# jin-s13/GKGNet

Measured on AMD Instinct MI355X. Metric: Grapher fwd+bwd images/sec, higher is better.
Workload: dtype f32; 1 GPU; BASELINE cfg2-literal: Grapher(C320,G4,k9,d1,18x18,relpos)+GrapherLabel(L80) fwd+bwd; batch_per_gpu=32, global_batch=32, C=320, G=4, HW=18x18, k=9, dilation=1, bn=local, parallelism=dp1, input_layout=nchw, launch=hipGraph replay of fwd+bwd+grad-pack, world_size=1, backend=none (single process), grad_allreduce=none (1 GPU)

## Files before the change

### gkgnet_amd/csrc/gkg_gemm_x6.hip

```cpp
#include "gkg_common.h"
#include <stdlib.h>
#include <vector>

namespace gkg {

typedef float x6_f32x16 __attribute__((ext_vector_type(16)));
typedef __attribute__((__vector_size__(8 * sizeof(__bf16)))) __bf16 x6_bf16x8;
typedef __bf16 x6_bf16x2 __attribute__((ext_vector_type(2)));
typedef float x6_f32x2 __attribute__((ext_vector_type(2)));

constexpr int X6_NPAD = 128;

__device__ __forceinline__ unsigned x6_cvt2(float a, float b) {
  x6_f32x2 v = {a, b};
  return __builtin_bit_cast(unsigned, __builtin_convertvector(v, x6_bf16x2));
}

__device__ __forceinline__ void x6_split2(float x0, float x1, unsigned& h, unsigned& m, unsigned& l) {
  h = x6_cvt2(x0, x1);
  const float r0 = x0 - __uint_as_float(h << 16), r1 = x1 - __uint_as_float(h & 0xffff0000u);
  m = x6_cvt2(r0, r1);
  const float s0 = r0 - __uint_as_float(m << 16), s1 = r1 - __uint_as_float(m & 0xffff0000u);
  l = x6_cvt2(s0, s1);
}
// ... 407 lines not shown
         ((flags & GKG_X6_FORCE_KS) || (nb == 1 && N <= 640));
}

static int x6_tile_ksplit(long long base2, int nk_total, bool has_ws) {
  if (!has_ws || base2 >= 320 || nk_total < 8) return 1;
  int ks = (int)(X6_SK_MAX_WG / base2);
  if (ks > nk_total / 4) ks = nk_total / 4;
  return ks > 8 ? 8 : ks;
}

template <int EPI>
static hipError_t x6_launch(X6Args a, int nb, hipStream_t st, void* sk_ws = nullptr, size_t sk_bytes = 0, unsigned flags = 0) {
  GkgProfScope prof(GKG_PROF_GEMM_X6, st, 2.0 * a.M * a.N * a.K * nb);
  const int mt = (a.M + 127) / 128;
  const long long base2 = (long long)mt * ((a.N + 63) / 64) * nb;
  const int nk_total = (a.K + 31) / 32;
  if constexpr (EPI != X6_STORE_NCHW) {
    if (x6_ks_form(a.M, a.N, nb, sk_ws != nullptr, flags)) {
      return x6_launch_ks<EPI, 1>(a, nb, st);
    }
  }
  if (const int ks = x6_tile_ksplit(base2, nk_total, sk_ws && sk_bytes >= X6_SK_BYTES); ks >= 2) {
    a.kper = (nk_total + ks - 1) / ks;
    a.ksplit = (nk_total + a.kper - 1) / a.kper;
    a.cnt = reinterpret_cast<unsigned*>(sk_ws);
    a.part = reinterpret_cast<float*>(reinterpret_cast<char*>(sk_ws) + X6_SK_CNT_BYTES);
    return x6_launch_ni<2, EPI>(a, nb, st);
  }
  if constexpr (EPI == X6_BNBWD) {
    if (a.add) return hipErrorInvalidValue;
  }
  int ni = base2 < 160 && !(flags & GKG_X6_FORCE_WALK) ? 1 : 2;
  if constexpr (EPI != X6_BNBWD && EPI != X6_STORE_NCHW) {
    if (a.N == 80 && ni == 2) return x6_launch_ni<3, EPI, 80>(a, nb, st);
  }
  if (ni == 1) return x6_launch_ni<1, EPI>(a, nb, st);
  if constexpr (EPI == X6_BNBWD) return x6_launch_ni<2, EPI>(a, nb, st);
  else return x6_launch_ni<2, EPI, 64, true>(a, nb, st, flags);
}

struct X6WgradArgs {
  const float* A;  size_t a_bstride;  int lda;
  const float* B;  size_t b_bstride;  int ldb;
  float* C;  size_t c_bstride;  int ldc;
  int M, N, K;
  int mtiles, ntiles, splits, rows_per_split;
  int swap;
  int share, rot;
  int ubase, urem;
  int kperm;
};

typedef unsigned x6_u32x4 __attribute__((ext_vector_type(4)));
typedef x6_u32x4 X6WFrag[4][3];

__device__ __forceinline__ x6_bf16x8 x6w_operand(const x6_u32x4& f) { return __builtin_bit_cast(x6_bf16x8, f); }
template <int I>
__device__ __forceinline__ void x6w_op(float (&raw)[4][8], X6WFrag& fn, unsigned (&t0)[4], unsigned (&t1)[4]) {
  constexpr int blk = I / 44, u = I % 44, p = u & 3, o = u >> 2;
  float& x0 = raw[blk][2 * p]; float& x1 = raw[blk][2 * p + 1];
  unsigned w;
  if constexpr (o == 0) { asm volatile("v_cvt_pk_bf16_f32 %0, %1, %2" : "=v"(w) : "v"(x0), "v"(x1)); fn[blk][0][p] = w; }
  if constexpr (o == 1) asm volatile("v_lshlrev_b32 %0, 16, %1" : "=v"(t0[p]) : "v"(fn[blk][0][p]));
  if constexpr (o == 2) asm volatile("v_and_b32 %0, 0xffff0000, %1" : "=v"(t1[p]) : "v"(fn[blk][0][p]));
  if constexpr (o == 3) asm volatile("v_sub_f32 %0, %0, %1" : "+v"(x0) : "v"(t0[p]));
  if constexpr (o == 4) asm volatile("v_sub_f32 %0, %0, %1" : "+v"(x1) : "v"(t1[p]));
  if constexpr (o == 5) { asm volatile("v_cvt_pk_bf16_f32 %0, %1, %2" : "=v"(w) : "v"(x0), "v"(x1)); fn[blk][1][p] = w; }
  if constexpr (o == 6) asm volatile("v_lshlrev_b32 %0, 16, %1" : "=v"(t0[p]) : "v"(fn[blk][1][p]));
  if constexpr (o == 7) asm volatile("v_and_b32 %0, 0xffff0000, %1" : "=v"(t1[p]) : "v"(fn[blk][1][p]));
  if constexpr (o == 8) asm volatile("v_sub_f32 %0, %0, %1" : "+v"(x0) : "v"(t0[p]));
  if constexpr (o == 9) asm volatile("v_sub_f32 %0, %0, %1" : "+v"(x1) : "v"(t1[p]));
  if constexpr (o == 10) { asm volatile("v_cvt_pk_bf16_f32 %0, %1, %2" : "=v"(w) : "v"(x0), "v"(x1)); fn[blk][2][p] = w; }
}
template <int I, int END>
__device__ __forceinline__ void x6w_ops(float (&raw)[4][8], X6WFrag& fn, unsigned (&t0)[4], unsigned (&t1)[4]) {
  if constexpr (I < END && I < 176) { x6w_op<I>(raw, fn, t0, t1); x6w_ops<I + 1, END>(raw, fn, t0, t1); }
}
template <int SI, bool SPLIT>
__device__ __forceinline__ void x6w_slots(const X6WFrag& fc, X6WFrag& fn, x6_f32x16 (&acc)[2][2], x6_f32x16 (&accs)[2][2],
                                          float (&raw)[4][8], unsigned (&t0)[4], unsigned (&t1)[4]) {
  if constexpr (SI < 24) {
    constexpr int i = SI / 12, j = (SI / 6) & 1, t = SI % 6;
    constexpr int pa = t == 0 ? 2 : (t == 2 || t == 3) ? 1 : 0;
    constexpr int pb = t == 1 ? 2 : (t == 2 || t == 4) ? 1 : 0;
    if constexpr (t < 5) accs[i][j] = __builtin_amdgcn_mfma_f32_32x32x16_bf16(x6w_operand(fc[i][pa]), x6w_operand(fc[2 + j][pb]), accs[i][j], 0, 0, 0);
    else acc[i][j] = __builtin_amdgcn_mfma_f32_32x32x16_bf16(x6w_operand(fc[i][0]), x6w_operand(fc[2 + j][0]), acc[i][j], 0, 0, 0);
    if constexpr (SPLIT) x6w_ops<SI * 8, SI * 8 + 8>(raw, fn, t0, t1);
    __builtin_amdgcn_sched_barrier(0);
    x6w_slots<SI + 1, SPLIT>(fc, fn, acc, accs, raw, t0, t1);
  }
}

#define X6W_DET 0
#include "gkg_wgrad_x6_rows.h"
#undef X6W_DET
#define X6W_DET 1
#include "gkg_wgrad_x6_rows.h"
#undef X6W_DET

__device__ __forceinline__ bool x6w_map(const X6WgradArgs& g, int lin, int& split, int& tile) {
  const int ntile = g.mtiles * g.ntiles;
  const int xcd = (lin + g.rot) & 7, slot = lin >> 3;
  if (g.share > 1) {
    split = xcd / g.share;
    tile = slot * g.share + xcd % g.share;
    return split < g.splits && tile < ntile;
  }
  split = (slot / ntile) * 8 + xcd;
  tile = slot % ntile;
  return split < g.splits;
}

template <bool DET>
__device__ __forceinline__ void wgrad_x6_dma_body(const X6WgradArgs& g, const int lin, const int z, const size_t sstride) {
  extern __shared__ float wlds[];
  const int tid = threadIdx.x, lane = tid & 63, w = __builtin_amdgcn_readfirstlane(tid >> 6);
  int split, tile;
  if (!x6w_map(g, lin, split, tile)) return;
  const int m0 = (tile / g.ntiles) * 64, n0 = (tile % g.ntiles) * 64;
  const int r = lane & 31, h = lane >> 5;
  const long long slab0 = 128ll * ((long long)split * g.ubase + min(split, g.urem));
  const int rows_here = 128 * (g.ubase + (split < g.urem ? 1 : 0));
  const int rows_per_wave = rows_here >> 2;
  const long long k_begin = slab0 + (long long)w * rows_per_wave;
  const int T = rows_per_wave >> 4;
  const char* Az = (const char*)(g.A + (size_t)z * g.a_bstride);
  const char* Bz = (const char*)(g.B + (size_t)z * g.b_bstride);
  const unsigned lds0 = (unsigned)(size_t)wlds + w * (4 * 8192);

  const int prow = lane >> 4, pch = lane & 15;
  const int ca = min(m0 + 4 * pch, g.M - 4), cb = min(n0 + 4 * pch, g.N - 4);
  const unsigned dA = (unsigned)(((size_t)prow * g.lda + ca) * 4), dB = (unsigned)(((size_t)prow * g.ldb + cb) * 4);
  const unsigned strideA = (unsigned)g.lda * 16u, strideB = (unsigned)g.ldb * 16u;
  auto dma = [&](int s) __attribute__((always_inline)) {
    const long long row0 = k_begin + 16ll * s;
    const char* ab = Az + row0 * g.lda * 4;
    const char* bb = Bz + row0 * g.ldb * 4;
    const unsigned dst = lds0 + (s & 3) * 8192;
#pragma unroll
    for (int p = 0; p < 4; ++p) {
      x6_dma16(ab, dA + p * strideA, dst + p * 1024);
      x6_dma16(bb, dB + p * strideB, dst + 4096 + p * 1024);
    }
  };
  const bool va0 = m0 + r < g.M, va1 = m0 + 32 + r < g.M, vb0 = n0 + r < g.N, vb1 = n0 + 32 + r < g.N;
  const bool tail = m0 + 64 > g.M || n0 + 64 > g.N;
  auto readfr = [&](float (&raw)[4][8], int s) __attribute__((always_inline)) {
    const float* base = wlds + w * (4 * 2048) + (s & 3) * 2048 + (8 * h) * 64 + r;
#pragma unroll
    for (int j = 0; j < 8; ++j) {
      raw[0][j] = base[j * 64];
      raw[1][j] = base[j * 64 + 32];
      raw[2][j] = base[1024 + j * 64];
      raw[3][j] = base[1024 + j * 64 + 32];
    }
    if (tail) {
#pragma unroll
      for (int j = 0; j < 8; ++j) {
        raw[0][j] = va0 ? raw[0][j] : 0.f; raw[1][j] = va1 ? raw[1][j] : 0.f;
        raw[2][j] = vb0 ? raw[2][j] : 0.f; raw[3][j] = vb1 ? raw[3][j] : 0.f;
      }
    }
  };
  float raw0[4][8], raw1[4][8];
  X6WFrag fr0, fr1;
  unsigned t0[4], t1[4];
  x6_f32x16 acc[2][2], accs[2][2];
#pragma unroll
  for (int i = 0; i < 2; ++i)
#pragma unroll
    for (int j = 0; j < 2; ++j)
#pragma unroll
      for (int q = 0; q < 16; ++q) { acc[i][j][q] = 0.f; accs[i][j][q] = 0.f; }

  dma(0);
  if (T > 1) dma(1);
  if (T > 2) dma(2);
  if (T > 3) dma(3);
  if (T > 3) asm volatile("s_waitcnt vmcnt(16)" ::: "memory");
  else asm volatile("s_waitcnt vmcnt(0)" ::: "memory");
  readfr(raw0, 0);
  if (T > 1) readfr(raw1, 1);
  x6w_ops<0, 176>(raw0, fr0, t0, t1);
  auto tailwork = [&](float (&rawn)[4][8], int s) __attribute__((always_inline)) {
    if (s + 4 < T) dma(s + 4);
    if (s + 2 < T) {
      if (s + 4 < T) asm volatile("s_waitcnt vmcnt(16)" ::: "memory");
      else if (s + 3 < T) asm volatile("s_waitcnt vmcnt(8)" ::: "memory");
      else asm volatile("s_waitcnt vmcnt(0)" ::: "memory");
      readfr(rawn, s + 2);
    }
  };
  for (int s = 0; s + 2 < T; s += 2) {
    x6w_slots<0, true>(fr0, fr1, acc, accs, raw1, t0, t1);
    tailwork(raw0, s);
    x6w_slots<0, true>(fr1, fr0, acc, accs, raw0, t0, t1);
    tailwork(raw1, s + 1);
  }
  x6w_slots<0, true>(fr0, fr1, acc, accs, raw1, t0, t1);
  x6w_slots<0, false>(fr1, fr0, acc, accs, raw0, t0, t1);
  asm volatile("s_waitcnt vmcnt(0)" ::: "memory");

  __syncthreads();
  float* red = wlds;
#pragma unroll
  for (int i = 0; i < 2; ++i)
#pragma unroll
    for (int j = 0; j < 2; ++j)
#pragma unroll
      for (int q = 0; q < 16; ++q) {
        const int row = 32 * i + (q & 3) + 8 * (q >> 2) + 4 * h, col = 32 * j + r;
        red[w * 4096 + row * 64 + col] = acc[i][j][q] + accs[i][j][q];
      }
  __syncthreads();
  float* C = g.C + (size_t)z * g.c_bstride;
#pragma unroll
  for (int u = 0; u < 16; ++u) {
    const int e = tid + 256 * u, row = e >> 6, col = e & 63;
    const float v = (red[e] + red[4096 + e]) + (red[8192 + e] + red[12288 + e]);
    if (m0 + row < g.M && n0 + col < g.N) {
      float* dst = C + (size_t)(m0 + row) * g.ldc + (g.kperm ? x6_kperm_src(n0 + col, g.N) : n0 + col);
      if constexpr (DET) dst[(size_t)split * sstride] = v;
      else __hip_atomic_fetch_add(dst, v, __ATOMIC_RELAXED, __HIP_MEMORY_SCOPE_AGENT);
    }
  }
}

__global__ __launch_bounds__(256) void wgrad_x6_dma_kernel(X6WgradArgs g) { wgrad_x6_dma_body<false>(g, blockIdx.x, blockIdx.y, 0); }
__global__ __launch_bounds__(256) void wgrad_x6_dma_det_kernel(X6WgradArgs g, size_t sstride) { wgrad_x6_dma_body<true>(g, blockIdx.x, blockIdx.y, sstride); }

typedef x6_u32x4 X6WFragW[6][3];

template <int I>
__device__ __forceinline__ void x6ww_op(float (&raw)[6][8], X6WFragW& fn, unsigned (&t0)[4], unsigned (&t1)[4]) {
  constexpr int blk = I / 44, u = I % 44, p = u & 3, o = u >> 2;
  float& x0 = raw[blk][2 * p]; float& x1 = raw[blk][2 * p + 1];
  unsigned w;
  if constexpr (o == 0) { asm volatile("v_cvt_pk_bf16_f32 %0, %1, %2" : "=v"(w) : "v"(x0), "v"(x1)); fn[blk][0][p] = w; }
  if constexpr (o == 1) asm volatile("v_lshlrev_b32 %0, 16, %1" : "=v"(t0[p]) : "v"(fn[blk][0][p]));
  if constexpr (o == 2) asm volatile("v_and_b32 %0, 0xffff0000, %1" : "=v"(t1[p]) : "v"(fn[blk][0][p]));
  if constexpr (o == 3) asm volatile("v_sub_f32 %0, %0, %1" : "+v"(x0) : "v"(t0[p]));
  if constexpr (o == 4) asm volatile("v_sub_f32 %0, %0, %1" : "+v"(x1) : "v"(t1[p]));
  if constexpr (o == 5) { asm volatile("v_cvt_pk_bf16_f32 %0, %1, %2" : "=v"(w) : "v"(x0), "v"(x1)); fn[blk][1][p] = w; }
  if constexpr (o == 6) asm volatile("v_lshlrev_b32 %0, 16, %1" : "=v"(t0[p]) : "v"(fn[blk][1][p]));
  if constexpr (o == 7) asm volatile("v_and_b32 %0, 0xffff0000, %1" : "=v"(t1[p]) : "v"(fn[blk][1][p]));
  if constexpr (o == 8) asm volatile("v_sub_f32 %0, %0, %1" : "+v"(x0) : "v"(t0[p]));
  if constexpr (o == 9) asm volatile("v_sub_f32 %0, %0, %1" : "+v"(x1) : "v"(t1[p]));
  if constexpr (o == 10) { asm volatile("v_cvt_pk_bf16_f32 %0, %1, %2" : "=v"(w) : "v"(x0), "v"(x1)); fn[blk][2][p] = w; }
}
template <int I, int END>
__device__ __forceinline__ void x6ww_ops(float (&raw)[6][8], X6WFragW& fn, unsigned (&t0)[4], unsigned (&t1)[4]) {
  if constexpr (I < END && I < 264) { x6ww_op<I>(raw, fn, t0, t1); x6ww_ops<I + 1, END>(raw, fn, t0, t1); }
}
template <int SI, bool SPLIT>
__device__ __forceinline__ void x6ww_slots(const X6WFragW& fc, X6WFragW& fn, x6_f32x16 (&acc)[2][4], float (&raw)[6][8],
                                           unsigned (&t0)[4], unsigned (&t1)[4]) {
  if constexpr (SI < 48) {
    constexpr int t = SI / 8, i = (SI % 8) / 4, j = SI % 4;
    constexpr int pa = t == 0 ? 2 : (t == 2 || t == 3) ? 1 : 0;
    constexpr int pb = t == 1 ? 2 : (t == 2 || t == 4) ? 1 : 0;
    acc[i][j] = __builtin_amdgcn_mfma_f32_32x32x16_bf16(x6w_operand(fc[i][pa]), x6w_operand(fc[2 + j][pb]), acc[i][j], 0, 0, 0);
    if constexpr (SPLIT) x6ww_ops<(SI * 11) / 2, ((SI + 1) * 11) / 2>(raw, fn, t0, t1);
    __builtin_amdgcn_sched_barrier(0);
    x6ww_slots<SI + 1, SPLIT>(fc, fn, acc, raw, t0, t1);
  }
}

template <bool DET>
__device__ __forceinline__ void wgrad_x6_wide_body(const X6WgradArgs& g, const int lin, const int z, const size_t sstride) {
  extern __shared__ float wlds[];
  constexpr int STAGE_BYTES = 16 * 192 * 4, STAGE_F = 16 * 192;
  const int tid = threadIdx.x, lane = tid & 63, w = __builtin_amdgcn_readfirstlane(tid >> 6);
  int split, tile;
  if (!x6w_map(g, lin, split, tile)) return;
  const int m0 = (tile / g.ntiles) * 64, n0 = (tile % g.ntiles) * 128;
  const int r = lane & 31, h = lane >> 5;
  const long long slab0 = 128ll * ((long long)split * g.ubase + min(split, g.urem));
  const int rows_here = 128 * (g.ubase + (split < g.urem ? 1 : 0));
  const int rows_per_wave = rows_here >> 2;
  const long long k_begin = slab0 + (long long)w * rows_per_wave;
  const int T = rows_per_wave >> 4;
  const char* Az = (const char*)(g.A + (size_t)z * g.a_bstride);
  const char* Bz = (const char*)(g.B + (size_t)z * g.b_bstride);
  const unsigned lds0 = (unsigned)(size_t)wlds + w * (3 * STAGE_BYTES);

  const int ca = min(m0 + 4 * (lane & 15), g.M - 4), cb = min(n0 + 4 * (lane & 31), g.N - 4);
  const unsigned dA = (unsigned)(((size_t)(lane >> 4) * g.lda + ca) * 4), dB = (unsigned)(((size_t)(lane >> 5) * g.ldb + cb) * 4);
  const unsigned strideA = (unsigned)g.lda * 16u, strideB = (unsigned)g.ldb * 8u;
  auto dma = [&](int s) __attribute__((always_inline)) {
    const long long row0 = k_begin + 16ll * s;
    const char* ab = Az + row0 * g.lda * 4;
    const char* bb = Bz + row0 * g.ldb * 4;
    const unsigned dst = lds0 + (s % 3) * STAGE_BYTES;
#pragma unroll
    for (int p = 0; p < 4; ++p) x6_dma16(ab, dA + p * strideA, dst + p * 1024);
#pragma unroll
    for (int p = 0; p < 8; ++p) x6_dma16(bb, dB + p * strideB, dst + 4096 + p * 1024);
  };
  bool va[2], vb[4];
#pragma unroll
  for (int i = 0; i < 2; ++i) va[i] = m0 + 32 * i + r < g.M;
#pragma unroll
  for (int j = 0; j < 4; ++j) vb[j] = n0 + 32 * j + r < g.N;
  const bool tail = m0 + 64 > g.M || n0 + 128 > g.N;
  auto readfr = [&](float (&raw)[6][8], int s) __attribute__((always_inline)) {
    const float* ba = wlds + w * (3 * STAGE_F) + (s % 3) * STAGE_F + (8 * h) * 64 + r;
    const float* bb = wlds + w * (3 * STAGE_F) + (s % 3) * STAGE_F + 1024 + (8 * h) * 128 + r;
#pragma unroll
    for (int j = 0; j < 8; ++j) {
      raw[0][j] = ba[j * 64];
      raw[1][j] = ba[j * 64 + 32];
#pragma unroll
      for (int q = 0; q < 4; ++q) raw[2 + q][j] = bb[j * 128 + 32 * q];
    }
    if (tail) {
#pragma unroll
      for (int j = 0; j < 8; ++j) {
        raw[0][j] = va[0] ? raw[0][j] : 0.f; raw[1][j] = va[1] ? raw[1][j] : 0.f;
#pragma unroll
        for (int q = 0; q < 4; ++q) raw[2 + q][j] = vb[q] ? raw[2 + q][j] : 0.f;
      }
    }
  };
  float raw0[6][8], raw1[6][8];
  X6WFragW fr0, fr1;
  unsigned t0[4], t1[4];
  x6_f32x16 acc[2][4];
#pragma unroll
  for (int i = 0; i < 2; ++i)
#pragma unroll
    for (int j = 0; j < 4; ++j)
#pragma unroll
      for (int q = 0; q < 16; ++q) acc[i][j][q] = 0.f;

  dma(0);
  dma(1);
  if (T > 2) dma(2);
  if (T > 2) asm volatile("s_waitcnt vmcnt(12)" ::: "memory");
  else asm volatile("s_waitcnt vmcnt(0)" ::: "memory");
  readfr(raw0, 0);
  readfr(raw1, 1);
  x6ww_ops<0, 264>(raw0, fr0, t0, t1);
  auto tailwork = [&](float (&rawn)[6][8], int s) __attribute__((always_inline)) {
    if (s + 3 < T) dma(s + 3);
    if (s + 2 < T) {
      if (s + 3 < T) asm volatile("s_waitcnt vmcnt(12)" ::: "memory");
      else asm volatile("s_waitcnt vmcnt(0)" ::: "memory");
      readfr(rawn, s + 2);
    }
  };
  for (int s = 0; s + 2 < T; s += 2) {
    x6ww_slots<0, true>(fr0, fr1, acc, raw1, t0, t1);
    tailwork(raw0, s);
    x6ww_slots<0, true>(fr1, fr0, acc, raw0, t0, t1);
    tailwork(raw1, s + 1);
  }
  x6ww_slots<0, true>(fr0, fr1, acc, raw1, t0, t1);
  x6ww_slots<0, false>(fr1, fr0, acc, raw0, t0, t1);
  asm volatile("s_waitcnt vmcnt(0)" ::: "memory");

  __syncthreads();
  float* red = wlds;
  constexpr int RP = 129, RW = 64 * RP;
#pragma unroll
  for (int i = 0; i < 2; ++i)
#pragma unroll
    for (int j = 0; j < 4; ++j)
#pragma unroll
      for (int q = 0; q < 16; ++q) {
        const int row = 32 * i + (q & 3) + 8 * (q >> 2) + 4 * h, col = 32 * j + r;
        red[w * RW + row * RP + col] = acc[i][j][q];
      }
  __syncthreads();
  float* C = g.C + (size_t)z * g.c_bstride;
#pragma unroll 4
  for (int u = 0; u < 32; ++u) {
    const int e = tid + 256 * u;
    const int row = g.swap ? (e & 63) : (e >> 7), col = g.swap ? (e >> 6) : (e & 127);
    const int o = row * RP + col;
    const float v = (red[o] + red[RW + o]) + (red[2 * RW + o] + red[3 * RW + o]);
    if (m0 + row < g.M && n0 + col < g.N) {
      const int wr = g.swap ? n0 + col : m0 + row, wc0 = g.swap ? m0 + row : n0 + col;
      const int wc = g.kperm ? x6_kperm_src(wc0, g.swap ? g.M : g.N) : wc0;
      float* dst = C + (size_t)wr * g.ldc + wc;
      if constexpr (DET) dst[(size_t)split * sstride] = v;
      else __hip_atomic_fetch_add(dst, v, __ATOMIC_RELAXED, __HIP_MEMORY_SCOPE_AGENT);
    }
  }
}

__global__ __launch_bounds__(256) void wgrad_x6_wide_kernel(X6WgradArgs g) { wgrad_x6_wide_body<false>(g, blockIdx.x, blockIdx.y, 0); }
__global__ __launch_bounds__(256) void wgrad_x6_wide_det_kernel(X6WgradArgs g, size_t sstride) { wgrad_x6_wide_body<true>(g, blockIdx.x, blockIdx.y, sstride); }

constexpr int X6W_BATCH = 16;
struct X6WgradBatch {
  int n;
  int begin[X6W_BATCH + 1];
  int gridx[X6W_BATCH];
  int wide[X6W_BATCH];
  X6WgradArgs p[X6W_BATCH];
};
// ... 302 lines not shown
                                            const float* residual, const float* py, const float* pa, const float* pc,
                                            const float* pmean, const float* pinvstd, double* psums, int pnb, int pco, int pact,
                                            void* splitk_ws, size_t splitk_bytes, unsigned flags, void* stream);
extern "C" int gkg_linear_dgrad_x6_bnbwd(const float* dy, int ldg, const void* planes_dgrad, float* dx, int R, int cin, int cout,
                                         const float* py, const float* pa, const float* pc, const float* pmean,
                                         const float* pinvstd, double* psums, int pnb, int pco, int pact, void* stream) {
  return gkg_linear_dgrad_x6_bnbwd_sk(dy, ldg, planes_dgrad, dx, R, cin, cout, nullptr, py, pa, pc, pmean, pinvstd, psums, pnb, pco, pact,
                                      nullptr, 0, 0, stream);
}

extern "C" int gkg_linear_dgrad_x6_bnbwd_sk_supported(int R, int cin, int has_residual, int has_ws, unsigned flags) {
  return (!has_residual || x6_ks_form(R, cin, 1, has_ws != 0, flags)) ? 1 : 0;
}

extern "C" int gkg_linear_dgrad_x6_bnbwd_sk(const float* dy, int ldg, const void* planes_dgrad, float* dx, int R, int cin, int cout,
                                            const float* residual, const float* py, const float* pa, const float* pc,
                                            const float* pmean, const float* pinvstd, double* psums, int pnb, int pco, int pact,
                                            void* splitk_ws, size_t splitk_bytes, unsigned flags, void* stream) {
  if (!dy || !planes_dgrad || !dx || !py || !pa || !pc || !pmean || !pinvstd || !psums)
    return gkg_fail(GKG_ERR_NULL, "gkg_linear_dgrad_x6_bnbwd_sk: null pointer");
  if (splitk_ws && (splitk_bytes < X6_SK_BYTES || ((size_t)splitk_ws & 15)))
    return gkg_fail(GKG_ERR_SHAPE, "gkg_linear_dgrad_x6_bnbwd_sk: need a 16-byte aligned workspace of gkg_x6_splitk_workspace_bytes() bytes (or NULL: no split)");
  if (R <= 0 || x6_bad_dim(cin) || x6_bad_dim(cout) || ldg < cout || (ldg & 3) || ((size_t)dy & 15) || pnb <= 0 || pco <= 0 ||
      (long long)pnb * pco != cin || (pact != 0 && pact != 1))
    return gkg_fail(GKG_ERR_SHAPE, "gkg_linear_dgrad_x6_bnbwd_sk: need R > 0, cin % 4 == 0, cout % 4 == 0, cin == pnb * pco, 16-byte aligned rows");
  if ((size_t)R * ldg * 4 > 0xffffffffull) return gkg_fail(GKG_ERR_UNSUPPORTED, "gkg_linear_dgrad_x6_bnbwd_sk: operand larger than 4 GiB");
  if (residual && !x6_ks_form(R, cin, 1, splitk_ws != nullptr, flags))
    return gkg_fail(GKG_ERR_UNSUPPORTED, "gkg_linear_dgrad_x6_bnbwd_sk: a residual needs the short-matrix body");
  X6Args a{};
  a.A = dy; a.a_bstride = 0; a.lda = ldg;
  a.NP = (cin + X6_NPAD - 1) / X6_NPAD * X6_NPAD; a.KC = (cout + 31) / 32 * 4;
  a.P = (const uint4*)planes_dgrad; a.p_bstride = (size_t)3 * a.KC * a.NP;
  a.C = dx; a.c_bstride = (size_t)R * cin; a.ldc = cin;
  a.M = R; a.N = cin; a.K = cout;
  a.add = residual;
  a.py = py; a.pa = pa; a.pc = pc; a.pmean = pmean; a.pinvstd = pinvstd; a.psums = psums; a.pco = pco; a.pact = pact;
  hipError_t e = x6_launch<X6_BNBWD>(a, 1, (hipStream_t)stream, splitk_ws, splitk_bytes, flags);
  return e == hipSuccess ? 0 : gkg_fail_hip(e, "gemm_x6 (dgrad + BN backward statistics)");
}

namespace gkg {
struct X6WgradPlan {
  X6WgradArgs main;
  bool wide;
  int grid_x;
  X6WgradArgs rest;
  int rest_grid_x;
};

static int x6_wgrad_set_attr(bool wide) {
  static bool once[3][64] = {};
  int dev = 0;
  (void)hipGetDevice(&dev);
  const size_t sh_w = (size_t)4 * 3 * 16 * 192 * 4, sh_d = (size_t)4 * 4 * 8192;
  if (dev < 0 || dev >= 64 || !once[wide][dev]) {
    hipError_t e = hipFuncSetAttribute(wide ? (const void*)wgrad_x6_wide_kernel : (const void*)wgrad_x6_dma_kernel,
                                       hipFuncAttributeMaxDynamicSharedMemorySize, (int)(wide ? sh_w : sh_d));
    if (e != hipSuccess) return gkg_fail_hip(e, "wgrad_x6 DMA kernel (attribute)");
    if (dev >= 0 && dev < 64) once[wide][dev] = true;
  }
  if (dev < 0 || dev >= 64 || !once[2][dev]) {
    hipError_t e = hipFuncSetAttribute((const void*)wgrad_x6_batch_kernel, hipFuncAttributeMaxDynamicSharedMemorySize, (int)sh_w);
    if (e != hipSuccess) return gkg_fail_hip(e, "wgrad_x6 batch kernel (attribute)");
    if (dev >= 0 && dev < 64) once[2][dev] = true;
  }
  return 0;
}

static int x6_wgrad_plan(const float* dy, int ldg, size_t g_bstride, const float* x, int ldx, size_t x_bstride, float* dw, int R,
                         int cin, int cout, int nb, int batched, X6WgradPlan& pl, int kperm = 0, int force_slabs = 0,
                         int aligned_as = -1) {
  if (!dy || !x || !dw) return gkg_fail(GKG_ERR_NULL, "gkg_linear_wgrad_x6: null pointer");
  if (kperm && (cin & 1)) return gkg_fail(GKG_ERR_SHAPE, "gkg_linear_wgrad_x6: kperm needs an even cin");
  if (R <= 0 || cin <= 0 || cout <= 0 || nb <= 0 || nb > 64 || ldg < cout || ldx < cin)
    return gkg_fail(GKG_ERR_SHAPE, "gkg_linear_wgrad_x6: need R, cin, cout > 0, 1 <= nb <= 64, pitches >= widths");
  if ((size_t)ldg * 4 * 16 > 0x7fffffffull || (size_t)ldx * 4 * 16 > 0x7fffffffull) return gkg_fail(GKG_ERR_UNSUPPORTED, "gkg_linear_wgrad_x6: row pitch too large");
  X6WgradArgs a{};
  a.A = dy; a.a_bstride = g_bstride; a.lda = ldg;
  a.B = x; a.b_bstride = x_bstride; a.ldb = ldx;
  a.C = dw; a.c_bstride = (size_t)cout * cin; a.ldc = cin;
  a.M = cout; a.N = cin; a.K = R;
  a.kperm = kperm ? 1 : 0;
  a.mtiles = (cout + 63) / 64; a.ntiles = (cin + 63) / 64;
  const bool aligned = (cin & 3) == 0 && (cout & 3) == 0 && (ldg & 3) == 0 && (ldx & 3) == 0 &&
                       (aligned_as >= 0 ? aligned_as != 0
                                        : (g_bstride & 3) == 0 && (x_bstride & 3) == 0 && ((size_t)dy & 15) == 0 && ((size_t)x & 15) == 0) &&
                       (size_t)R * ldg * 4 < 0xffffffffull && (size_t)R * ldx * 4 < 0xffffffffull;
  const long long padn = (long long)((cin + 127) / 128) * 128 * 100 / ((long long)a.ntiles * 64);
  const long long padm = (long long)((cout + 127) / 128) * 128 * 100 / ((long long)a.mtiles * 64);
  bool wide = aligned && (padn <= 110 || padm <= 110);
  bool swap = wide && padm < padn;
  if (batched > 0 && aligned) {
    const long long c64 = (long long)a.mtiles * a.ntiles * 36;
    const long long cwn = (long long)a.mtiles * ((cin + 127) / 128) * 48, cwm = (long long)a.ntiles * ((cout + 127) / 128) * 48;
    wide = (cwn < cwm ? cwn : cwm) <= c64;
    swap = wide && cwm < cwn;
  }
  const int main_mtiles = !wide ? a.mtiles : (swap ? a.ntiles : a.mtiles);
  const int main_ntiles = !wide ? a.ntiles : (swap ? (cout + 127) / 128 : (cin + 127) / 128);
  const int tiles = main_mtiles * main_ntiles * nb, units = R / 128;
  int splits = 1, share = 0;
  int sp_alone = 1;
  {
    long long best = -1;
    for (int sp = 1; sp <= units && sp <= 4096; ++sp) {
      const long long per_xcd = (long long)tiles * ((sp + 7) / 8);
      const long long rounds = (per_xcd + 31) / 32;
// ... 14 lines not shown
    splits = force_slabs > 0 ? force_slabs : sp_alone;
  }
  a.rows_per_split = units > 0 ? (units + splits - 1) / splits * 128 : 128;
  const int main_rows = aligned ? units * 128 : 0;
  pl.wide = wide;
  pl.main = a;
  pl.main.K = 0;
  pl.grid_x = 0;
  if (main_rows > 0) {
    X6WgradArgs m = a;
    m.mtiles = main_mtiles; m.ntiles = main_ntiles;
    if (swap) {
      m.A = x; m.a_bstride = x_bstride; m.lda = ldx; m.M = cin;
      m.B = dy; m.b_bstride = g_bstride; m.ldb = ldg; m.N = cout;
      m.swap = 1;
    }
    m.K = main_rows; m.splits = splits < units ? splits : units;
    m.ubase = units / m.splits; m.urem = units % m.splits;
    if (share > 1 && m.splits * share == 8) {
      m.share = share;
      pl.grid_x = (m.mtiles * m.ntiles + share - 1) / share * 8;
    } else {
      pl.grid_x = (m.splits + 7) / 8 * 8 * m.mtiles * m.ntiles;
    }
    pl.main = m;
  }
  const int done = main_rows, rest = R - done;
  pl.rest = a;
  pl.rest.K = 0;
  pl.rest_grid_x = 0;
  if (rest > 0) {
    X6WgradArgs t = a;
    t.A = dy + (size_t)done * ldg; t.B = x + (size_t)done * ldx; t.K = rest;
    const int tunits = (rest + 127) / 128;
    int ts = splits > tunits ? tunits : splits;
    t.rows_per_split = (tunits + ts - 1) / ts * 128;
    t.splits = (rest + t.rows_per_split - 1) / t.rows_per_split;
    pl.rest = t;
    pl.rest_grid_x = (t.splits + 7) / 8 * 8 * a.mtiles * a.ntiles;
  }
  return 0;
}
}

extern "C" int gkg_linear_wgrad_x6(const float* dy, int ldg, size_t g_bstride, const float* x, int ldx, size_t x_bstride,
                                   float* dw, int R, int cin, int cout, int nb, int kperm, void* stream) {
  X6WgradPlan pl;
  int rc = x6_wgrad_plan(dy, ldg, g_bstride, x, ldx, x_bstride, dw, R, cin, cout, nb, 0, pl, kperm);
  if (rc) return rc;
  hipStream_t st = (hipStream_t)stream;
  hipError_t e = hipSuccess;
  if (pl.main.K > 0) {
    if ((rc = x6_wgrad_set_attr(pl.wide))) return rc;
    const size_t sh = pl.wide ? (size_t)4 * 3 * 16 * 192 * 4 : (size_t)4 * 4 * 8192;
    const dim3 grid(pl.grid_x, nb);
    if (pl.wide) hipLaunchKernelGGL(wgrad_x6_wide_kernel, grid, dim3(256), sh, st, pl.main);
    else hipLaunchKernelGGL(wgrad_x6_dma_kernel, grid, dim3(256), sh, st, pl.main);
    e = hipGetLastError();
    if (e != hipSuccess) return gkg_fail_hip(e, "wgrad_x6 DMA kernel");
  }
  if (pl.rest.K > 0) {
    hipLaunchKernelGGL(wgrad_x6_kernel, dim3(pl.rest_grid_x, nb), dim3(256), 0, st, pl.rest);
    e = hipGetLastError();
  }
  return e == hipSuccess ? 0 : gkg_fail_hip(e, "wgrad_x6_kernel");
}

extern "C" int gkg_linear_wgrad_x6_batch(const GkgWgradProblem* p, int n, int units_per_slab, void* stream) {
  if (!p || n <= 0) return gkg_fail(GKG_ERR_NULL, "gkg_linear_wgrad_x6_batch: no problems");
  if (units_per_slab < 0 || units_per_slab > 4096) return gkg_fail(GKG_ERR_SHAPE, "gkg_linear_wgrad_x6_batch: units_per_slab out of range");
  if (units_per_slab == 0) units_per_slab = 20;
  hipStream_t st = (hipStream_t)stream;
  int order[256];
  if (n > 256) return gkg_fail(GKG_ERR_SHAPE, "gkg_linear_wgrad_x6_batch: at most 256 problems per call");
  for (int i = 0; i < n; ++i) order[i] = i;
  auto work = [&](int i) { return (double)p[i].R * p[i].cin * p[i].cout * p[i].nb; };
  for (int i = 1; i < n; ++i)
    for (int j = i; j > 0 && work(order[j]) > work(order[j - 1]); --j) { const int t = order[j]; order[j] = order[j - 1]; order[j - 1] = t; }
  X6WgradBatch b{};
  int rot = 0;
  auto flush = [&]() -> int {
    if (b.n == 0) return 0;
    int rc = x6_wgrad_set_attr(true);
    if (rc) return rc;
    hipLaunchKernelGGL(wgrad_x6_batch_kernel, dim3(b.begin[b.n]), dim3(256), (size_t)4 * 3 * 16 * 192 * 4, st, b);
    hipError_t e = hipGetLastError();
    b.n = 0;
    return e == hipSuccess ? 0 : gkg_fail_hip(e, "wgrad_x6_batch_kernel");
  };
  for (int oi = 0; oi < n; ++oi) {
    const GkgWgradProblem& q = p[order[oi]];
    X6WgradPlan pl;
    int rc = x6_wgrad_plan(q.dy, q.ldg, q.g_bstride, q.x, q.ldx, q.x_bstride, q.dw, q.R, q.cin, q.cout, q.nb, units_per_slab, pl, q.kperm);
    if (rc) return rc;
    if (pl.main.K > 0) {
      const int i = b.n;
      pl.main.rot = rot;
      rot = (rot + (pl.main.share > 1 ? 0 : pl.main.splits)) & 7;
      b.p[i] = pl.main; b.wide[i] = pl.wide ? 1 : 0; b.gridx[i] = pl.grid_x;
      b.begin[i + 1] = b.begin[i] + pl.grid_x * q.nb;
      b.n = i + 1;
      if (b.n == X6W_BATCH && (rc = flush())) return rc;
    }
    if (pl.rest.K > 0) {
      hipLaunchKernelGGL(wgrad_x6_kernel, dim3(pl.rest_grid_x, q.nb), dim3(256), 0, st, pl.rest);
      hipError_t e = hipGetLastError();
      if (e != hipSuccess) return gkg_fail_hip(e, "wgrad_x6_kernel");
    }
  }
  return flush();
}

namespace gkg {
constexpr size_t X6W_SH_WIDE = (size_t)4 * 3 * 16 * 192 * 4, X6W_SH_DMA = (size_t)4 * 4 * 8192;

static int x6_wdet_set_attr(int kind) {
  static bool once[3][64] = {};
  int dev = 0;
  (void)hipGetDevice(&dev);
  if (dev < 0 || dev >= 64 || !once[kind][dev]) {
    const void* f = kind == 0 ? (const void*)wgrad_x6_dma_det_kernel
                              : kind == 1 ? (const void*)wgrad_x6_wide_det_kernel : (const void*)wgrad_x6_batch_det_kernel;
    hipError_t e = hipFuncSetAttribute(f, hipFuncAttributeMaxDynamicSharedMemorySize, (int)(kind == 0 ? X6W_SH_DMA : X6W_SH_WIDE));
    if (e != hipSuccess) return gkg_fail_hip(e, "wgrad_x6 deterministic kernel (attribute)");
    if (dev >= 0 && dev < 64) once[kind][dev] = true;
  }
  return 0;
}

inline int x6_wdet_main_slabs(const X6WgradPlan& pl) { return pl.main.K > 0 ? pl.main.splits : 0; }
inline int x6_wdet_slabs(const X6WgradPlan& pl) { return x6_wdet_main_slabs(pl) + (pl.rest.K > 0 ? pl.rest.splits : 0); }
inline bool x6_wdet_elems_ok(int cin, int cout, int nb) {
  return cin > 0 && cout > 0 && nb > 0 && (unsigned long long)nb * (unsigned long long)cout * (unsigned long long)cin <= (1ull << 31);
}
static const float* const X6W_ANY = reinterpret_cast<const float*>(16);

struct X6WdetReducer {
  X6WdetReduce d{};
  hipStream_t st;
  int flush() {
    if (d.n == 0) return 0;
    hipLaunchKernelGGL(wgrad_x6_det_reduce_kernel, dim3(d.begin[d.n]), dim3(256), 0, st, d);
    hipError_t e = hipGetLastError();
    d.n = 0;
    return e == hipSuccess ? 0 : gkg_fail_hip(e, "wgrad_x6_det_reduce_kernel");
  }
  int add(float* dw, const float* ws, size_t E, int S) {
    const long long blocks = (long long)((E + 255) / 256);
    if (d.n == X6W_BATCH || (d.n > 0 && (long long)d.begin[d.n] + blocks > 0x7fffffffll)) {
      int rc = flush();
      if (rc) return rc;
    }
    const int i = d.n;
    d.dw[i] = dw; d.ws[i] = ws; d.E[i] = E; d.S[i] = S;
    d.begin[i + 1] = d.begin[i] + (int)blocks;
    d.n = i + 1;
    return 0;
  }
};
}

extern "C" size_t gkg_linear_wgrad_x6_det_workspace_bytes(int R, int cin, int cout, int nb, int ldg, int ldx, int slabs) {
  if (slabs < 0 || slabs > 4096 || !x6_wdet_elems_ok(cin, cout, nb)) return 0;
  int S = 0;
  for (int al = 0; al < 2; ++al) {
    X6WgradPlan pl;
    if (x6_wgrad_plan(X6W_ANY, ldg, 0, X6W_ANY, ldx, 0, const_cast<float*>(X6W_ANY), R, cin, cout, nb, 0, pl, 0, slabs, al)) return 0;
    const int s = x6_wdet_slabs(pl);
// ... 161 lines not shown
```

Before: 40200 images/s.

## Rework wgrad DMA ring addressing, zero-page masking and fine-grained LDS waits

The wgrad DMA and wide kernels now issue the global-to-LDS loads through one inline-asm sequence that bumps m0, and advance incrementally updated row pointers and ring write/read offsets instead of recomputing addresses per stage. Out-of-range tail lanes read from a small zeroed LDS page rather than applying per-element select masks. LDS fragment reads use ds_read2st64 asm, and staggered lgkmcnt waits are inserted so the bf16 split conversion can start on each block before all reads land. The change costs 4 KB of extra shared memory per block and a __syncthreads, and the hand-written waitcnt counts must match the real number of outstanding LDS reads.

```diff
diff --git a/gkgnet_amd/csrc/gkg_gemm_x6.hip b/gkgnet_amd/csrc/gkg_gemm_x6.hip
--- a/gkgnet_amd/csrc/gkg_gemm_x6.hip
+++ b/gkgnet_amd/csrc/gkg_gemm_x6.hip
@@ -483,14 +483,20 @@
 };
 
 typedef unsigned x6_u32x4 __attribute__((ext_vector_type(4)));
+typedef float x6_f32x2 __attribute__((ext_vector_type(2)));
 typedef x6_u32x4 X6WFrag[4][3];
+typedef x6_u32x4 X6WFragW[6][3];
 
 __device__ __forceinline__ x6_bf16x8 x6w_operand(const x6_u32x4& f) { return __builtin_bit_cast(x6_bf16x8, f); }
-template <int I>
-__device__ __forceinline__ void x6w_op(float (&raw)[4][8], X6WFrag& fn, unsigned (&t0)[4], unsigned (&t1)[4]) {
+template <int I, int NB, bool LDSW>
+__device__ __forceinline__ void x6w_op(float (&raw)[NB][8], x6_u32x4 (&fn)[NB][3], unsigned (&t0)[4], unsigned (&t1)[4]) {
   constexpr int blk = I / 44, u = I % 44, p = u & 3, o = u >> 2;
   float& x0 = raw[blk][2 * p]; float& x1 = raw[blk][2 * p + 1];
   unsigned w;
+  if constexpr (LDSW && u == 0) {
+    constexpr int left = 4 * (NB - 1 - blk);
+    asm volatile("s_waitcnt lgkmcnt(%0)" :: "n"(left < 15 ? left : 15) : "memory");
+  }
   if constexpr (o == 0) { asm volatile("v_cvt_pk_bf16_f32 %0, %1, %2" : "=v"(w) : "v"(x0), "v"(x1)); fn[blk][0][p] = w; }
   if constexpr (o == 1) asm volatile("v_lshlrev_b32 %0, 16, %1" : "=v"(t0[p]) : "v"(fn[blk][0][p]));
   if constexpr (o == 2) asm volatile("v_and_b32 %0, 0xffff0000, %1" : "=v"(t1[p]) : "v"(fn[blk][0][p]));
@@ -503,11 +509,11 @@
   if constexpr (o == 9) asm volatile("v_sub_f32 %0, %0, %1" : "+v"(x1) : "v"(t1[p]));
   if constexpr (o == 10) { asm volatile("v_cvt_pk_bf16_f32 %0, %1, %2" : "=v"(w) : "v"(x0), "v"(x1)); fn[blk][2][p] = w; }
 }
-template <int I, int END>
-__device__ __forceinline__ void x6w_ops(float (&raw)[4][8], X6WFrag& fn, unsigned (&t0)[4], unsigned (&t1)[4]) {
-  if constexpr (I < END && I < 176) { x6w_op<I>(raw, fn, t0, t1); x6w_ops<I + 1, END>(raw, fn, t0, t1); }
-}
-template <int SI, bool SPLIT>
+template <int I, int END, bool LDSW = false, int NB>
+__device__ __forceinline__ void x6w_ops(float (&raw)[NB][8], x6_u32x4 (&fn)[NB][3], unsigned (&t0)[4], unsigned (&t1)[4]) {
+  if constexpr (I < END && I < 44 * NB) { x6w_op<I, NB, LDSW>(raw, fn, t0, t1); x6w_ops<I + 1, END, LDSW>(raw, fn, t0, t1); }
+}
+template <int SI, bool SPLIT, bool LDSW = false>
 __device__ __forceinline__ void x6w_slots(const X6WFrag& fc, X6WFrag& fn, x6_f32x16 (&acc)[2][2], x6_f32x16 (&accs)[2][2],
                                           float (&raw)[4][8], unsigned (&t0)[4], unsigned (&t1)[4]) {
   if constexpr (SI < 24) {
@@ -516,9 +522,9 @@
     constexpr int pb = t == 1 ? 2 : (t == 2 || t == 4) ? 1 : 0;
     if constexpr (t < 5) accs[i][j] = __builtin_amdgcn_mfma_f32_32x32x16_bf16(x6w_operand(fc[i][pa]), x6w_operand(fc[2 + j][pb]), accs[i][j], 0, 0, 0);
     else acc[i][j] = __builtin_amdgcn_mfma_f32_32x32x16_bf16(x6w_operand(fc[i][0]), x6w_operand(fc[2 + j][0]), acc[i][j], 0, 0, 0);
-    if constexpr (SPLIT) x6w_ops<SI * 8, SI * 8 + 8>(raw, fn, t0, t1);
+    if constexpr (SPLIT) x6w_ops<SI * 8, SI * 8 + 8, LDSW>(raw, fn, t0, t1);
     __builtin_amdgcn_sched_barrier(0);
-    x6w_slots<SI + 1, SPLIT>(fc, fn, acc, accs, raw, t0, t1);
+    x6w_slots<SI + 1, SPLIT, LDSW>(fc, fn, acc, accs, raw, t0, t1);
   }
 }
 
@@ -540,6 +546,32 @@
   split = (slot / ntile) * 8 + xcd;
   tile = slot % ntile;
   return split < g.splits;
+}
+
+constexpr unsigned X6W_ZERO_BYTES = 4096;
+constexpr size_t X6W_SH_DMA = (size_t)4 * 4 * 8192 + X6W_ZERO_BYTES, X6W_SH_WIDE = (size_t)4 * 3 * 16 * 192 * 4 + X6W_ZERO_BYTES;
+
+__device__ __forceinline__ void x6w_dma4(const void* sbase, unsigned v0, unsigned v1, unsigned v2, unsigned v3, unsigned lds_dst) {
+  unsigned keep;
+  asm volatile("s_mov_b32 %0, m0\n\ts_mov_b32 m0, %6\n\ts_nop 0\n\tglobal_load_lds_dwordx4 %1, %5\n\t"
+               "s_add_u32 m0, m0, 0x400\n\ts_nop 0\n\tglobal_load_lds_dwordx4 %2, %5\n\t"
+               "s_add_u32 m0, m0, 0x400\n\ts_nop 0\n\tglobal_load_lds_dwordx4 %3, %5\n\t"
+               "s_add_u32 m0, m0, 0x400\n\ts_nop 0\n\tglobal_load_lds_dwordx4 %4, %5\n\t"
+               "s_mov_b32 m0, %0"
+               : "=&s"(keep) : "v"(v0), "v"(v1), "v"(v2), "v"(v3), "s"(sbase), "s"(lds_dst) : "memory", "scc");
+}
+template <int PB>
+__device__ __forceinline__ void x6w_readblk(float (&f)[8], unsigned addr) {
+  x6_f32x2 v0, v1, v2, v3;
+  asm volatile("ds_read2st64_b32 %0, %1 offset0:%2 offset1:%3" : "=v"(v0) : "v"(addr), "n"(0), "n"(PB) : "memory");
+  asm volatile("ds_read2st64_b32 %0, %1 offset0:%2 offset1:%3" : "=v"(v1) : "v"(addr), "n"(2 * PB), "n"(3 * PB) : "memory");
+  asm volatile("ds_read2st64_b32 %0, %1 offset0:%2 offset1:%3" : "=v"(v2) : "v"(addr), "n"(4 * PB), "n"(5 * PB) : "memory");
+  asm volatile("ds_read2st64_b32 %0, %1 offset0:%2 offset1:%3" : "=v"(v3) : "v"(addr), "n"(6 * PB), "n"(7 * PB) : "memory");
+  f[0] = v0.x; f[1] = v0.y; f[2] = v1.x; f[3] = v1.y; f[4] = v2.x; f[5] = v2.y; f[6] = v3.x; f[7] = v3.y;
+}
+__device__ __forceinline__ void x6w_clear_zero(float* wlds, unsigned ring_bytes, int tid) {
+  static_assert(X6W_ZERO_BYTES == 256 * 16, "one 16-byte store per thread");
+  reinterpret_cast<float4*>(wlds + ring_bytes / 4)[tid] = float4{0.f, 0.f, 0.f, 0.f};
 }
 
 template <bool DET>
@@ -557,41 +589,39 @@
   const int T = rows_per_wave >> 4;
   const char* Az = (const char*)(g.A + (size_t)z * g.a_bstride);
   const char* Bz = (const char*)(g.B + (size_t)z * g.b_bstride);
-  const unsigned lds0 = (unsigned)(size_t)wlds + w * (4 * 8192);
+  constexpr unsigned RING_BYTES = 4 * 4 * 8192;
+  const unsigned lds_base = (unsigned)(size_t)wlds;
+  const unsigned lds0 = lds_base + w * (4 * 8192), lds_end = lds0 + 4 * 8192, lds_zero = lds_base + RING_BYTES;
+  x6w_clear_zero(wlds, RING_BYTES, tid);
 
   const int prow = lane >> 4, pch = lane & 15;
   const int ca = min(m0 + 4 * pch, g.M - 4), cb = min(n0 + 4 * pch, g.N - 4);
   const unsigned dA = (unsigned)(((size_t)prow * g.lda + ca) * 4), dB = (unsigned)(((size_t)prow * g.ldb + cb) * 4);
   const unsigned strideA = (unsigned)g.lda * 16u, strideB = (unsigned)g.ldb * 16u;
-  auto dma = [&](int s) __attribute__((always_inline)) {
-    const long long row0 = k_begin + 16ll * s;
-    const char* ab = Az + row0 * g.lda * 4;
-    const char* bb = Bz + row0 * g.ldb * 4;
-    const unsigned dst = lds0 + (s & 3) * 8192;
-#pragma unroll
-    for (int p = 0; p < 4; ++p) {
-      x6_dma16(ab, dA + p * strideA, dst + p * 1024);
-      x6_dma16(bb, dB + p * strideB, dst + 4096 + p * 1024);
-    }
+  unsigned va[4], vb[4];
+#pragma unroll
+  for (int p = 0; p < 4; ++p) { va[p] = dA + p * strideA; vb[p] = dB + p * strideB; }
+  const char* arow = Az + k_begin * g.lda * 4;
+  const char* brow = Bz + k_begin * g.ldb * 4;
+  const size_t stepA = (size_t)g.lda * 64, stepB = (size_t)g.ldb * 64;
+  unsigned wr = lds0;
+  auto dma = [&]() __attribute__((always_inline)) {
+    x6w_dma4(arow, va[0], va[1], va[2], va[3], wr);
+    x6w_dma4(brow, vb[0], vb[1], vb[2], vb[3], wr + 4096);
+    arow += stepA; brow += stepB;
+    wr += 8192;
+    if (wr == lds_end) wr = lds0;
   };
-  const bool va0 = m0 + r < g.M, va1 = m0 + 32 + r < g.M, vb0 = n0 + r < g.N, vb1 = n0 + 32 + r < g.N;
-  const bool tail = m0 + 64 > g.M || n0 + 64 > g.N;
-  auto readfr = [&](float (&raw)[4][8], int s) __attribute__((always_inline)) {
-    const float* base = wlds + w * (4 * 2048) + (s & 3) * 2048 + (8 * h) * 64 + r;
-#pragma unroll
-    for (int j = 0; j < 8; ++j) {
-      raw[0][j] = base[j * 64];
-      raw[1][j] = base[j * 64 + 32];
-      raw[2][j] = base[1024 + j * 64];
-      raw[3][j] = base[1024 + j * 64 + 32];
-    }
-    if (tail) {
-#pragma unroll
-      for (int j = 0; j < 8; ++j) {
-        raw[0][j] = va0 ? raw[0][j] : 0.f; raw[1][j] = va1 ? raw[1][j] : 0.f;
-        raw[2][j] = vb0 ? raw[2][j] : 0.f; raw[3][j] = vb1 ? raw[3][j] : 0.f;
-      }
-    }
+  const bool ok[4] = {m0 + r < g.M, m0 + 32 + r < g.M, n0 + r < g.N, n0 + 32 + r < g.N};
+  unsigned lo[4];
+#pragma unroll
+  for (int q = 0; q < 4; ++q) lo[q] = (unsigned)(((q >> 1) * 1024 + (8 * h) * 64 + 32 * (q & 1) + r) * 4);
+  unsigned rd = lds0;
+  auto readfr = [&](float (&raw)[4][8]) __attribute__((always_inline)) {
+#pragma unroll
+    for (int q = 0; q < 4; ++q) x6w_readblk<1>(raw[q], ok[q] ? rd + lo[q] : lds_zero);
+    rd += 8192;
+    if (rd == lds_end) rd = lds0;
   };
   float raw0[4][8], raw1[4][8];
   X6WFrag fr0, fr1;
@@ -604,31 +634,32 @@
 #pragma unroll
       for (int q = 0; q < 16; ++q) { acc[i][j][q] = 0.f; accs[i][j][q] = 0.f; }
 
-  dma(0);
-  if (T > 1) dma(1);
-  if (T > 2) dma(2);
-  if (T > 3) dma(3);
+  dma();
+  if (T > 1) dma();
+  if (T > 2) dma();
+  if (T > 3) dma();
+  __syncthreads();
   if (T > 3) asm volatile("s_waitcnt vmcnt(16)" ::: "memory");
   else asm volatile("s_waitcnt vmcnt(0)" ::: "memory");
-  readfr(raw0, 0);
-  if (T > 1) readfr(raw1, 1);
-  x6w_ops<0, 176>(raw0, fr0, t0, t1);
+  readfr(raw0);
+  if (T > 1) readfr(raw1);
+  x6w_ops<0, 176, true>(raw0, fr0, t0, t1);
   auto tailwork = [&](float (&rawn)[4][8], int s) __attribute__((always_inline)) {
-    if (s + 4 < T) dma(s + 4);
+    if (s + 4 < T) dma();
     if (s + 2 < T) {
       if (s + 4 < T) asm volatile("s_waitcnt vmcnt(16)" ::: "memory");
       else if (s + 3 < T) asm volatile("s_waitcnt vmcnt(8)" ::: "memory");
       else asm volatile("s_waitcnt vmcnt(0)" ::: "memory");
-      readfr(rawn, s + 2);
+      readfr(rawn);
     }
   };
   for (int s = 0; s + 2 < T; s += 2) {
-    x6w_slots<0, true>(fr0, fr1, acc, accs, raw1, t0, t1);
+    x6w_slots<0, true, true>(fr0, fr1, acc, accs, raw1, t0, t1);
     tailwork(raw0, s);
-    x6w_slots<0, true>(fr1, fr0, acc, accs, raw0, t0, t1);
+    x6w_slots<0, true, true>(fr1, fr0, acc, accs, raw0, t0, t1);
     tailwork(raw1, s + 1);
   }
-  x6w_slots<0, true>(fr0, fr1, acc, accs, raw1, t0, t1);
+  x6w_slots<0, true, true>(fr0, fr1, acc, accs, raw1, t0, t1);
   x6w_slots<0, false>(fr1, fr0, acc, accs, raw0, t0, t1);
   asm volatile("s_waitcnt vmcnt(0)" ::: "memory");
 
@@ -660,29 +691,7 @@
 __global__ __launch_bounds__(256) void wgrad_x6_dma_kernel(X6WgradArgs g) { wgrad_x6_dma_body<false>(g, blockIdx.x, blockIdx.y, 0); }
 __global__ __launch_bounds__(256) void wgrad_x6_dma_det_kernel(X6WgradArgs g, size_t sstride) { wgrad_x6_dma_body<true>(g, blockIdx.x, blockIdx.y, sstride); }
 
-typedef x6_u32x4 X6WFragW[6][3];
-
-template <int I>
-__device__ __forceinline__ void x6ww_op(float (&raw)[6][8], X6WFragW& fn, unsigned (&t0)[4], unsigned (&t1)[4]) {
-  constexpr int blk = I / 44, u = I % 44, p = u & 3, o = u >> 2;
-  float& x0 = raw[blk][2 * p]; float& x1 = raw[blk][2 * p + 1];
-  unsigned w;
-  if constexpr (o == 0) { asm volatile("v_cvt_pk_bf16_f32 %0, %1, %2" : "=v"(w) : "v"(x0), "v"(x1)); fn[blk][0][p] = w; }
-  if constexpr (o == 1) asm volatile("v_lshlrev_b32 %0, 16, %1" : "=v"(t0[p]) : "v"(fn[blk][0][p]));
-  if constexpr (o == 2) asm volatile("v_and_b32 %0, 0xffff0000, %1" : "=v"(t1[p]) : "v"(fn[blk][0][p]));
-  if constexpr (o == 3) asm volatile("v_sub_f32 %0, %0, %1" : "+v"(x0) : "v"(t0[p]));
-  if constexpr (o == 4) asm volatile("v_sub_f32 %0, %0, %1" : "+v"(x1) : "v"(t1[p]));
-  if constexpr (o == 5) { asm volatile("v_cvt_pk_bf16_f32 %0, %1, %2" : "=v"(w) : "v"(x0), "v"(x1)); fn[blk][1][p] = w; }
-  if constexpr (o == 6) asm volatile("v_lshlrev_b32 %0, 16, %1" : "=v"(t0[p]) : "v"(fn[blk][1][p]));
-  if constexpr (o == 7) asm volatile("v_and_b32 %0, 0xffff0000, %1" : "=v"(t1[p]) : "v"(fn[blk][1][p]));
-  if constexpr (o == 8) asm volatile("v_sub_f32 %0, %0, %1" : "+v"(x0) : "v"(t0[p]));
-  if constexpr (o == 9) asm volatile("v_sub_f32 %0, %0, %1" : "+v"(x1) : "v"(t1[p]));
-  if constexpr (o == 10) { asm volatile("v_cvt_pk_bf16_f32 %0, %1, %2" : "=v"(w) : "v"(x0), "v"(x1)); fn[blk][2][p] = w; }
-}
-template <int I, int END>
-__device__ __forceinline__ void x6ww_ops(float (&raw)[6][8], X6WFragW& fn, unsigned (&t0)[4], unsigned (&t1)[4]) {
-  if constexpr (I < END && I < 264) { x6ww_op<I>(raw, fn, t0, t1); x6ww_ops<I + 1, END>(raw, fn, t0, t1); }
-}
+
 template <int SI, bool SPLIT>
 __device__ __forceinline__ void x6ww_slots(const X6WFragW& fc, X6WFragW& fn, x6_f32x16 (&acc)[2][4], float (&raw)[6][8],
                                            unsigned (&t0)[4], unsigned (&t1)[4]) {
@@ -691,7 +700,7 @@
     constexpr int pa = t == 0 ? 2 : (t == 2 || t == 3) ? 1 : 0;
     constexpr int pb = t == 1 ? 2 : (t == 2 || t == 4) ? 1 : 0;
     acc[i][j] = __builtin_amdgcn_mfma_f32_32x32x16_bf16(x6w_operand(fc[i][pa]), x6w_operand(fc[2 + j][pb]), acc[i][j], 0, 0, 0);
-    if constexpr (SPLIT) x6ww_ops<(SI * 11) / 2, ((SI + 1) * 11) / 2>(raw, fn, t0, t1);
+    if constexpr (SPLIT) x6w_ops<(SI * 11) / 2, ((SI + 1) * 11) / 2, true>(raw, fn, t0, t1);
     __builtin_amdgcn_sched_barrier(0);
     x6ww_slots<SI + 1, SPLIT>(fc, fn, acc, raw, t0, t1);
   }
@@ -713,45 +722,45 @@
   const int T = rows_per_wave >> 4;
   const char* Az = (const char*)(g.A + (size_t)z * g.a_bstride);
   const char* Bz = (const char*)(g.B + (size_t)z * g.b_bstride);
-  const unsigned lds0 = (unsigned)(size_t)wlds + w * (3 * STAGE_BYTES);
+  constexpr unsigned RING_BYTES = 4 * 3 * STAGE_BYTES;
+  const unsigned lds_base = (unsigned)(size_t)wlds;
+  const unsigned lds0 = lds_base + w * (3 * STAGE_BYTES), lds_end = lds0 + 3 * STAGE_BYTES, lds_zero = lds_base + RING_BYTES;
+  x6w_clear_zero(wlds, RING_BYTES, tid);
 
   const int ca = min(m0 + 4 * (lane & 15), g.M - 4), cb = min(n0 + 4 * (lane & 31), g.N - 4);
   const unsigned dA = (unsigned)(((size_t)(lane >> 4) * g.lda + ca) * 4), dB = (unsigned)(((size_t)(lane >> 5) * g.ldb + cb) * 4);
   const unsigned strideA = (unsigned)g.lda * 16u, strideB = (unsigned)g.ldb * 8u;
-  auto dma = [&](int s) __attribute__((always_inline)) {
-    const long long row0 = k_begin + 16ll * s;
-    const char* ab = Az + row0 * g.lda * 4;
-    const char* bb = Bz + row0 * g.ldb * 4;
-    const unsigned dst = lds0 + (s % 3) * STAGE_BYTES;
-#pragma unroll
-    for (int p = 0; p < 4; ++p) x6_dma16(ab, dA + p * strideA, dst + p * 1024);
-#pragma unroll
-    for (int p = 0; p < 8; ++p) x6_dma16(bb, dB + p * strideB, dst + 4096 + p * 1024);
+  unsigned va[4], vb[8];
+#pragma unroll
+  for (int p = 0; p < 4; ++p) va[p] = dA + p * strideA;
+#pragma unroll
+  for (int p = 0; p < 8; ++p) vb[p] = dB + p * strideB;
+  const char* arow = Az + k_begin * g.lda * 4;
+  const char* brow = Bz + k_begin * g.ldb * 4;
+  const size_t stepA = (size_t)g.lda * 64, stepB = (size_t)g.ldb * 64;
+  unsigned wr = lds0;
+  auto dma = [&]() __attribute__((always_inline)) {
+    x6w_dma4(arow, va[0], va[1], va[2], va[3], wr);
+    x6w_dma4(brow, vb[0], vb[1], vb[2], vb[3], wr + 4096);
+    x6w_dma4(brow, vb[4], vb[5], vb[6], vb[7], wr + 8192);
+    arow += stepA; brow += stepB;
+    wr += STAGE_BYTES;
+    if (wr == lds_end) wr = lds0;
   };
-  bool va[2], vb[4];
-#pragma unroll
-  for (int i = 0; i < 2; ++i) va[i] = m0 + 32 * i + r < g.M;
-#pragma unroll
-  for (int j = 0; j < 4; ++j) vb[j] = n0 + 32 * j + r < g.N;
-  const bool tail = m0 + 64 > g.M || n0 + 128 > g.N;
-  auto readfr = [&](float (&raw)[6][8], int s) __attribute__((always_inline)) {
-    const float* ba = wlds + w * (3 * STAGE_F) + (s % 3) * STAGE_F + (8 * h) * 64 + r;
-    const float* bb = wlds + w * (3 * STAGE_F) + (s % 3) * STAGE_F + 1024 + (8 * h) * 128 + r;
-#pragma unroll
-    for (int j = 0; j < 8; ++j) {
-      raw[0][j] = ba[j * 64];
-      raw[1][j] = ba[j * 64 + 32];
-#pragma unroll
-      for (int q = 0; q < 4; ++q) raw[2 + q][j] = bb[j * 128 + 32 * q];
-    }
-    if (tail) {
-#pragma unroll
-      for (int j = 0; j < 8; ++j) {
-        raw[0][j] = va[0] ? raw[0][j] : 0.f; raw[1][j] = va[1] ? raw[1][j] : 0.f;
-#pragma unroll
-        for (int q = 0; q < 4; ++q) raw[2 + q][j] = vb[q] ? raw[2 + q][j] : 0.f;
-      }
-    }
+  bool ok[6];
+  unsigned lo[6];
+#pragma unroll
+  for (int q = 0; q < 2; ++q) { ok[q] = m0 + 32 * q + r < g.M; lo[q] = (unsigned)(((8 * h) * 64 + 32 * q + r) * 4); }
+#pragma unroll
+  for (int q = 0; q < 4; ++q) { ok[2 + q] = n0 + 32 * q + r < g.N; lo[2 + q] = (unsigned)((1024 + (8 * h) * 128 + 32 * q + r) * 4); }
+  unsigned rd = lds0;
+  auto readfr = [&](float (&raw)[6][8]) __attribute__((always_inline)) {
+#pragma unroll
+    for (int q = 0; q < 2; ++q) x6w_readblk<1>(raw[q], ok[q] ? rd + lo[q] : lds_zero);
+#pragma unroll
+    for (int q = 2; q < 6; ++q) x6w_readblk<2>(raw[q], ok[q] ? rd + lo[q] : lds_zero);
+    rd += STAGE_BYTES;
+    if (rd == lds_end) rd = lds0;
   };
   float raw0[6][8], raw1[6][8];
   X6WFragW fr0, fr1;
@@ -764,20 +773,21 @@
 #pragma unroll
       for (int q = 0; q < 16; ++q) acc[i][j][q] = 0.f;
 
-  dma(0);
-  dma(1);
-  if (T > 2) dma(2);
+  dma();
+  dma();
+  if (T > 2) dma();
+  __syncthreads();
   if (T > 2) asm volatile("s_waitcnt vmcnt(12)" ::: "memory");
   else asm volatile("s_waitcnt vmcnt(0)" ::: "memory");
-  readfr(raw0, 0);
-  readfr(raw1, 1);
-  x6ww_ops<0, 264>(raw0, fr0, t0, t1);
+  readfr(raw0);
+  readfr(raw1);
+  x6w_ops<0, 264, true>(raw0, fr0, t0, t1);
   auto tailwork = [&](float (&rawn)[6][8], int s) __attribute__((always_inline)) {
-    if (s + 3 < T) dma(s + 3);
+    if (s + 3 < T) dma();
     if (s + 2 < T) {
       if (s + 3 < T) asm volatile("s_waitcnt vmcnt(12)" ::: "memory");
       else asm volatile("s_waitcnt vmcnt(0)" ::: "memory");
-      readfr(rawn, s + 2);
+      readfr(rawn);
     }
   };
   for (int s = 0; s + 2 < T; s += 2) {
@@ -1186,7 +1196,7 @@
   static bool once[3][64] = {};
   int dev = 0;
   (void)hipGetDevice(&dev);
-  const size_t sh_w = (size_t)4 * 3 * 16 * 192 * 4, sh_d = (size_t)4 * 4 * 8192;
+  const size_t sh_w = X6W_SH_WIDE, sh_d = X6W_SH_DMA;
   if (dev < 0 || dev >= 64 || !once[wide][dev]) {
     hipError_t e = hipFuncSetAttribute(wide ? (const void*)wgrad_x6_wide_kernel : (const void*)wgrad_x6_dma_kernel,
                                        hipFuncAttributeMaxDynamicSharedMemorySize, (int)(wide ? sh_w : sh_d));
@@ -1307,7 +1317,7 @@
   hipError_t e = hipSuccess;
   if (pl.main.K > 0) {
     if ((rc = x6_wgrad_set_attr(pl.wide))) return rc;
-    const size_t sh = pl.wide ? (size_t)4 * 3 * 16 * 192 * 4 : (size_t)4 * 4 * 8192;
+    const size_t sh = pl.wide ? X6W_SH_WIDE : X6W_SH_DMA;
     const dim3 grid(pl.grid_x, nb);
     if (pl.wide) hipLaunchKernelGGL(wgrad_x6_wide_kernel, grid, dim3(256), sh, st, pl.main);
     else hipLaunchKernelGGL(wgrad_x6_dma_kernel, grid, dim3(256), sh, st, pl.main);
@@ -1338,7 +1348,7 @@
     if (b.n == 0) return 0;
     int rc = x6_wgrad_set_attr(true);
     if (rc) return rc;
-    hipLaunchKernelGGL(wgrad_x6_batch_kernel, dim3(b.begin[b.n]), dim3(256), (size_t)4 * 3 * 16 * 192 * 4, st, b);
+    hipLaunchKernelGGL(wgrad_x6_batch_kernel, dim3(b.begin[b.n]), dim3(256), X6W_SH_WIDE, st, b);
     hipError_t e = hipGetLastError();
     b.n = 0;
     return e == hipSuccess ? 0 : gkg_fail_hip(e, "wgrad_x6_batch_kernel");
@@ -1367,8 +1377,6 @@
 }
 
 namespace gkg {
-constexpr size_t X6W_SH_WIDE = (size_t)4 * 3 * 16 * 192 * 4, X6W_SH_DMA = (size_t)4 * 4 * 8192;
-
 static int x6_wdet_set_attr(int kind) {
   static bool once[3][64] = {};
   int dev = 0;
```

Result: faster. 40910 images/s, median of 6 (+1.7%).
